# sreeramkannan/Shannon

Hardware: AMD Instinct MI355X
Metric: reads/sec k-mer->graph->path-decompose, 2x100bp k=25 (higher is better)
Workload: dtype u64

## Files before the change

### include/shannon_hip.h

```cpp
#ifndef SHANNON_HIP_H
#define SHANNON_HIP_H
#include <stdint.h>
#ifdef __cplusplus
extern "C" {
#endif

typedef struct shn_ctx shn_ctx;
typedef struct shn_reads shn_reads;
typedef struct shn_table shn_table;

#define SHN_OK 0
#define SHN_ERR_ARG -1
#define SHN_ERR_HIP -2
#define SHN_ERR_NOMEM -3
#define SHN_ERR_OVERFLOW -4
#define SHN_ERR_INTERNAL -5

#define SHN_ENC_ASCII 0
#define SHN_ENC_CODES 1

const char* shn_last_error(void);
const char* shn_version(void);

int shn_ctx_create(int device, void* stream, shn_ctx** out);
// ... 5 lines not shown
int shn_timer_reset(shn_ctx* ctx);
int shn_timer_ms(shn_ctx* ctx, int slot, double* ms, uint64_t* n_regions);
int shn_timer_bytes(shn_ctx* ctx, int slot, uint64_t* bytes);
const char* shn_timer_name(int slot);

int shn_reads_create(shn_ctx* ctx, const uint8_t* bytes, const uint64_t* offsets, uint64_t n_reads,
                     uint32_t fixed_len, int enc, shn_reads** out);
void shn_reads_destroy(shn_reads* r);
uint64_t shn_reads_count(const shn_reads* r);
uint64_t shn_reads_total_bases(const shn_reads* r);
uint32_t shn_reads_max_len(const shn_reads* r);
uint64_t shn_reads_n_invalid(const shn_reads* r);

int shn_string_windows(const uint8_t* text, const uint64_t* off, uint64_t n_strings, int k, uint64_t* keys_out, uint8_t* rows_out);

int shn_gather_rows(const uint8_t* src, uint64_t n_src_rows, uint64_t row_bytes, const int64_t* idx, uint64_t n, uint8_t* dst, int threads);
int shn_gather_segments(const uint8_t* src, const uint64_t* src_off, uint64_t n_src, const int64_t* order, uint64_t n, uint8_t* dst,
                        const uint64_t* dst_off, int threads);
int shn_fasta_records(const uint8_t* src, const uint64_t* src_off, uint64_t n_src, const int64_t* order, uint64_t n, const char* prefix,
                      uint8_t* dst, uint64_t dst_cap, uint64_t* dst_len);

int shn_count_k1mers(shn_ctx* ctx, shn_reads* const* sets, int n_sets, int k1, int both_strands,
                     shn_table** out);
void shn_table_destroy(shn_table* t);
uint64_t shn_table_size(const shn_table* t);
uint64_t shn_table_total(const shn_table* t);
int shn_table_k(const shn_table* t);
int shn_table_canonical(const shn_table* t);
int shn_table_download(shn_ctx* ctx, const shn_table* t, uint64_t* keys, uint32_t* counts);
int shn_table_dump(shn_ctx* ctx, const shn_table* t, uint32_t lower, uint64_t* keys, uint32_t* counts,
                   uint64_t* n);
int shn_table_filter_lower(shn_ctx* ctx, const shn_table* t, uint32_t lower, shn_table** out);
int shn_table_device_ptrs(const shn_table* t, void** keys, void** counts);
int shn_table_lookup(shn_ctx* ctx, const shn_table* t, const uint64_t* keys, uint64_t n, uint32_t* counts);

int shn_table_from_pairs(shn_ctx* ctx, const void* dev_keys, const void* dev_counts, uint64_t n, int k1,
                         int canonical, shn_table** out);
int shn_table_merge_rc(shn_ctx* ctx, const shn_table* fwd, const shn_table* other, shn_table** out);
int shn_table_shard(shn_ctx* ctx, const shn_table* t, int n_ranks, uint64_t* per_rank, void* dev_keys_out,
                    void* dev_counts_out);
int shn_table_shard_mode(shn_ctx* ctx, const shn_table* t, int n_ranks, int mode, uint64_t* per_rank, void* dev_keys_out,
                         void* dev_counts_out);

typedef struct shn_ext shn_ext;
int shn_extend(shn_ctx* ctx, const shn_table* t, uint32_t min_weight, int max_iterations, shn_ext** out);
void shn_ext_destroy(shn_ext* e);
uint64_t shn_ext_n_walks(const shn_ext* e);
int shn_ext_iterations(const shn_ext* e);
uint64_t shn_ext_total_steps(const shn_ext* e);
uint64_t shn_ext_wave_steps(const shn_ext* e);
uint64_t shn_ext_fresh_steps(const shn_ext* e);
int shn_ext_dense_rounds(const shn_ext* e);
uint64_t shn_ext_settled_walks(const shn_ext* e);
int shn_ext_digests(const shn_ext* e, uint64_t* out );
uint64_t shn_debug_counter(int which);
int shn_debug_alloc(shn_ctx* ctx, uint64_t bytes, void** out);
void shn_debug_free(shn_ctx* ctx, void* p);
int shn_debug_fill(shn_ctx* ctx, void* p, uint64_t n_words, uint32_t value, uint32_t spin);
int shn_debug_read(shn_ctx* ctx, const void* p, uint64_t n_words, uint32_t* host_out);
int shn_ext_stats(shn_ctx* ctx, const shn_ext* e, uint32_t* n_right, uint32_t* n_left, uint64_t* tot_weight);
int shn_ext_stats_range(shn_ctx* ctx, const shn_ext* e, uint64_t lo, uint64_t n, uint32_t* n_right, uint32_t* n_left, uint64_t* tot_weight);
typedef void (*shn_block_cb)(void* user, shn_ext* ext, uint64_t lo, uint64_t hi, int status);
void shn_ext_set_block_callback(shn_block_cb cb, void* user);
int shn_ext_emit(shn_ctx* ctx, const shn_ext* e, const uint32_t* ranks, uint64_t n_sel, const uint64_t* offsets,
                 uint8_t* bases_out);
int shn_ext_weights(shn_ctx* ctx, const shn_ext* e, const uint64_t* keys, uint64_t n, uint32_t* weights);
// ... 165 lines not shown
```

### shannon_amd/_lib.py

```python
import ctypes as C
import os

_PKG = os.path.dirname(os.path.abspath(__file__))
LIB_PATH = os.environ.get("SHN_HIP_LIB") or os.path.join(_PKG, "libshannon_hip.so")
_lib = None

u8p, u32p, u64p, dblp = C.POINTER(C.c_uint8), C.POINTER(C.c_uint32), C.POINTER(C.c_uint64), C.POINTER(C.c_double)
vp, vpp = C.c_void_p, C.POINTER(C.c_void_p)

SIGNATURES = {
    "shn_last_error": (C.c_char_p, []),
    "shn_version": (C.c_char_p, []),
    "shn_ctx_create": (C.c_int, [C.c_int, vp, vpp]),
    "shn_ctx_destroy": (None, [vp]),
    "shn_ctx_sync": (C.c_int, [vp]),
    "shn_ctx_fork": (C.c_int, [vp, vpp]),
    "shn_ctx_own_workspaces": (C.c_int, [vp]),
    "shn_timer_reset": (C.c_int, [vp]),
    "shn_timer_ms": (C.c_int, [vp, C.c_int, dblp, u64p]),
    "shn_timer_bytes": (C.c_int, [vp, C.c_int, u64p]),
    "shn_timer_name": (C.c_char_p, [C.c_int]),
    "shn_reads_create": (C.c_int, [vp, vp, vp, C.c_uint64, C.c_uint32, C.c_int, vpp]),
    "shn_reads_destroy": (None, [vp]),
    "shn_reads_count": (C.c_uint64, [vp]),
    "shn_reads_total_bases": (C.c_uint64, [vp]),
    "shn_reads_max_len": (C.c_uint32, [vp]),
    "shn_reads_n_invalid": (C.c_uint64, [vp]),
    "shn_string_windows": (C.c_int, [vp, vp, C.c_uint64, C.c_int, vp, vp]),
    "shn_gather_rows": (C.c_int, [vp, C.c_uint64, C.c_uint64, vp, C.c_uint64, vp, C.c_int]),
    "shn_gather_segments": (C.c_int, [vp, vp, C.c_uint64, vp, C.c_uint64, vp, vp, C.c_int]),
    "shn_fasta_records": (C.c_int, [vp, vp, C.c_uint64, vp, C.c_uint64, C.c_char_p, vp, C.c_uint64, u64p]),
    "shn_count_k1mers": (C.c_int, [vp, vpp, C.c_int, C.c_int, C.c_int, vpp]),
    "shn_table_destroy": (None, [vp]),
    "shn_table_size": (C.c_uint64, [vp]),
    "shn_table_total": (C.c_uint64, [vp]),
    "shn_table_k": (C.c_int, [vp]),
    "shn_table_canonical": (C.c_int, [vp]),
    "shn_table_download": (C.c_int, [vp, vp, vp, vp]),
    "shn_table_dump": (C.c_int, [vp, vp, C.c_uint32, vp, vp, u64p]),
    "shn_table_filter_lower": (C.c_int, [vp, vp, C.c_uint32, vpp]),
    "shn_table_device_ptrs": (C.c_int, [vp, vpp, vpp]),
    "shn_table_lookup": (C.c_int, [vp, vp, vp, C.c_uint64, vp]),
    "shn_table_from_pairs": (C.c_int, [vp, vp, vp, C.c_uint64, C.c_int, C.c_int, vpp]),
    "shn_table_merge_rc": (C.c_int, [vp, vp, vp, vpp]),
    "shn_table_shard": (C.c_int, [vp, vp, C.c_int, u64p, vp, vp]),
    "shn_table_shard_mode": (C.c_int, [vp, vp, C.c_int, C.c_int, u64p, vp, vp]),
    "shn_debug_cc_counters": (C.c_int, [u64p, C.c_int]),
    "shn_cc_create": (C.c_int, [vp, vp, C.c_int, C.c_int, vpp]),
    "shn_cc_destroy": (None, [vp]),
    "shn_cc_query_counts": (C.c_int, [vp, u64p]),
    "shn_cc_queries": (C.c_int, [vp, vp, vp]),
    "shn_cc_answer": (C.c_int, [vp, vp, vp, u64p, u64p, vp, u64p]),
    "shn_cc_solve": (C.c_int, [vp, vp, C.c_uint64, C.c_uint64, vp, vp, u64p]),
    "shn_cc_labels": (C.c_int, [vp, C.c_uint64, vp, vp, C.c_uint64, vp]),
    "shn_cc_owners": (C.c_int, [vp, vp, vp, vp, C.c_uint64, vp]),
    "shn_cc_shard": (C.c_int, [vp, vp, u64p, vp, vp]),
    "shn_table_create": (C.c_int, [vp, vp, vp, C.c_uint64, C.c_int, C.c_int, vpp]),
    "shn_probe_build": (C.c_int, [vp, vp, vp, C.c_uint64, vp, C.c_uint32, C.c_int, vpp]),
    "shn_probe_destroy": (None, [vp]),
    "shn_probe_table": (vp, [vp]),
    "shn_probe_n_sets": (C.c_uint32, [vp]),
    "shn_probe_n_members": (C.c_uint64, [vp]),
    "shn_probe_sets": (C.c_int, [vp, vp, vp]),
    "shn_route_reads": (C.c_int, [vp, vp, vp, C.c_int, vp, vp, vp, C.c_uint32, vpp]),
    "shn_route_reads_mode": (C.c_int, [vp, vp, vp, C.c_int, vp, vp, vp, C.c_uint32, C.c_int, vpp]),
    "shn_routes_destroy": (None, [vp]),
    "shn_routes_size": (C.c_uint64, [vp]),
    "shn_routes_download": (C.c_int, [vp, vp, vp, vp]),
    "shn_routes_bounds": (C.c_int, [vp, vp, C.c_uint32, C.c_uint32, vp, vp]),
    "shn_routes_download_range": (C.c_int, [vp, vp, C.c_uint64, C.c_uint64, vp]),
    "shn_lp_solve_batch": (C.c_int, [vp, C.c_uint32, vp, vp, vp, vp, vp, vp, C.c_uint64, vp]),
    "shn_lp_set_rule": (C.c_int, [vp, C.c_int]),
    "shn_lp_stats": (C.c_int, [vp, vp, C.c_int]),
    "shn_contig_graph": (C.c_int, [vp, vp, C.c_uint64, C.c_int, C.c_int, C.c_double, vp, u64p, vp, vp, vp, u64p]),
# ... 170 lines not shown
```

### shannon_amd/csrc/count.hip

```cpp
#include "common.h"
#include <mutex>
#include <atomic>
#include <thread>
#include <functional>
#include <cmath>
#include <algorithm>
#include <cstring>

#define BLK 256
#define CAP 1024
#define CAP_LIMIT 950
#define TARGET_BUCKET 640
#define TILE_IDS 65536
#define TILE_KEYS 32768
#define EMPTY_KEY 0xFFFFFFFFFFFFFFFFULL

#include "count_views.h"

#define bucket_of shn_bucket_of

template <bool CANON>
__device__ __forceinline__ bool gen_key(const ReadsView& v, uint64_t r, uint32_t pos, int k, uint64_t& key) {
  uint32_t len = v.len ? v.len[r] : v.fixed_len;
  if (pos + k > len) return false;
// ... 907 lines not shown
  ShnDevBufs bufs(s);
  uint32_t* d_flag = nullptr; uint64_t* d_pos = nullptr;
  HIP_TRY(bufs.get(&d_flag, (n + 1) * 4)); HIP_TRY(bufs.get(&d_pos, (n + 2) * 8));
  const dim3 grid((uint32_t)std::max<uint64_t>(1, std::min<uint64_t>(cdiv(n, 256), 1u << 20))), blk(256);
  if (n) hipLaunchKernelGGL(table_keep_kernel, grid, blk, 0, s, (const uint64_t*)t->d_keys, (const uint32_t*)t->d_counts, n, t->k, t->canonical, lower, d_flag);
  uint64_t kept = 0;
  if (n) { int rc = shn_device_scan_u32(ctx, d_flag, n, d_pos, &kept); if (rc) return rc; }
  else HIP_TRY(hipMemsetAsync(d_pos, 0, 16, s));
  shn_table* o = new shn_table();
  *o = *t;
  o->ctx = ctx; o->n = kept; o->d_keys = nullptr; o->d_counts = nullptr; o->d_bucket_off = nullptr;
#define TRYT(x) do { hipError_t _e = (x); if (_e != hipSuccess) { shn_table_destroy(o); return shn_fail(SHN_ERR_HIP, std::string(#x) + ": " + hipGetErrorString(_e)); } } while (0)
  TRYT(shn_dev_malloc(&o->d_keys, (kept + 1) * 8));
  TRYT(shn_dev_malloc(&o->d_counts, (kept + 1) * 4));
  TRYT(shn_dev_malloc(&o->d_bucket_off, nb1 * 8));
  if (n) hipLaunchKernelGGL(table_keep_scatter_kernel, grid, blk, 0, s, (const uint64_t*)t->d_keys, (const uint32_t*)t->d_counts, (const uint32_t*)d_flag,
                            (const uint64_t*)d_pos, n, o->d_keys, o->d_counts);
  hipLaunchKernelGGL(table_keep_boff_kernel, dim3((uint32_t)std::min<uint64_t>(cdiv(nb1, 256), 1u << 20)), blk, 0, s, (const uint64_t*)t->d_bucket_off, nb1,
                     (const uint64_t*)d_pos, o->d_bucket_off);
  TRYT(hipGetLastError());
  TRYT(hipStreamSynchronize(s));
#undef TRYT
  *out = o;
  return SHN_OK;
}

extern "C" int shn_table_device_ptrs(const shn_table* t, void** keys, void** counts) {
  if (!t) return shn_fail(SHN_ERR_ARG, "shn_table_device_ptrs: NULL table");
  if (keys) *keys = t->d_keys;
  if (counts) *counts = t->d_counts;
  return SHN_OK;
}

extern "C" int shn_table_lookup(shn_ctx* ctx, const shn_table* t, const uint64_t* keys, uint64_t n, uint32_t* counts) {
  if (!ctx || !t || (!keys && n) || (!counts && n)) return shn_fail(SHN_ERR_ARG, "shn_table_lookup: NULL argument");
  if (!n) return SHN_OK;
  SHN_ENTER(ctx);
  hipStream_t s = ctx->stream; shn_use_stream(s);
  uint64_t* dq; uint32_t* dc;
  HIP_TRY(shn_hip_malloc(&dq, n * 8));
  HIP_TRY(shn_hip_malloc(&dc, n * 4));
  HIP_TRY(hipMemcpyAsync(dq, keys, n * 8, hipMemcpyHostToDevice, s));
  {
    TimerRegion tr(ctx, T_LOOKUP);
    hipLaunchKernelGGL(lookup_kernel, dim3((uint32_t)cdiv(n, 256)), dim3(256), 0, s, shn_tab_idx(t), t->d_counts, dq, n, dc);
  }
  HIP_TRY(hipMemcpyAsync(counts, dc, n * 4, hipMemcpyDeviceToHost, s));
  HIP_TRY(hipStreamSynchronize(s));
  hipFree(dq); hipFree(dc);
  return SHN_OK;
}

__global__ void sum_counts_kernel(const uint32_t* __restrict__ c, uint64_t n, unsigned long long* __restrict__ out) {
  unsigned long long a = 0;
  for (uint64_t i = (uint64_t)blockIdx.x * blockDim.x + threadIdx.x; i < n; i += (uint64_t)gridDim.x * blockDim.x) a += c[i];
  for (int o = 32; o > 0; o >>= 1) a += __shfl_down(a, o, 64);
  if ((threadIdx.x & 63) == 0 && a) atomicAdd(out, a);
}

__global__ void table_rc_concat_kernel(const uint64_t* __restrict__ ka, const uint32_t* __restrict__ ca, uint64_t na, const uint64_t* __restrict__ kb,
                                       const uint32_t* __restrict__ cb, uint64_t nb, int k, uint64_t* __restrict__ keys, uint32_t* __restrict__ cnts) {
  for (uint64_t i = (uint64_t)blockIdx.x * blockDim.x + threadIdx.x; i < na + nb; i += (uint64_t)gridDim.x * blockDim.x) {
    if (i < na) { keys[i] = ka[i]; cnts[i] = ca[i]; }
    else { keys[i] = shn_revcomp(kb[i - na], k); cnts[i] = cb[i - na]; }
  }
}
// ... 156 lines not shown
```

### shannon_amd/csrc/extend.hip

```cpp
#include "common.h"
#include <cstring>
#include <vector>
#include <time.h>
#include <cstdio>
#include <cstdlib>
#include <algorithm>

#define EBLK 256
#define WBLK 64
#define UNCLAIMED 0xFFFFFFFFu
#define NONE32 0xFFFFFFFFu
#define UNCLAIMED64 0xFFFFFFFFFFFFFFFFULL
#define NOHINT_WORD 0xFFFFFFFFu
#define LONG_WALK 8
#define MEMO_MIN 1
#define PROMOTE_STEPS 16
typedef unsigned long long u64;
#define CLAIM(rank, pos) (((u64)(rank) << 32) | (u64)(uint32_t)(pos))
#define RANK(c) ((uint32_t)((c) >> 32))
#define POS(c) ((uint32_t)(c))

struct Adj4 { int32_t v[4]; };
struct __attribute__((aligned(64))) Rec {
  Adj4 R;
// ... 81 lines not shown
#define FD_SLOTS 10
#define FD_PER_LINE 4
#define FD_HOPS 4
#define FD_PAL 0x80000000u
__device__ __forceinline__ uint64_t fd_bucket(const TabIdx& T, uint64_t key, uint64_t n_lines) {
  const uint64_t h = shn_mix64(key);
  if (!T.layout) return __umul64hi(h, n_lines);
  const uint32_t b = shn_tab_bucket(T, key);
  const uint64_t lo = T.boff[b], hi = T.boff[b + 1];
  return lo / FD_PER_LINE + b + __umul64hi(h, (hi - lo) / FD_PER_LINE + 1);
}
__device__ __forceinline__ uint64_t fd_line_in_bucket(const TabIdx& T, uint32_t b, uint64_t key) {
  const uint64_t lo = T.boff[b], hi = T.boff[b + 1];
  return lo / FD_PER_LINE + b + __umul64hi(shn_mix64(key), (hi - lo) / FD_PER_LINE + 1);
}
__device__ __forceinline__ uint64_t xcd_block(int on) {
  const uint32_t g8 = gridDim.x & ~7u;
  if (!on || blockIdx.x >= g8) return blockIdx.x;
  return (uint64_t)(blockIdx.x & 7u) * (g8 >> 3) + (blockIdx.x >> 3);
}
__global__ void fd_build_kernel(const TabIdx T, const uint8_t* __restrict__ flags, uint64_t n,
                                unsigned long long* __restrict__ lines, uint64_t n_lines, int xcd) {
  const uint64_t* __restrict__ tkeys = T.keys;
  const uint64_t i = xcd_block(xcd) * blockDim.x + threadIdx.x;
  if (i >= n) return;
  const uint8_t f = flags[i];
  if (f & 2) return;
  const uint64_t key = tkeys[i];
  unsigned long long* line = lines + fd_bucket(T, key, n_lines) * 16;
  for (int hop = 0; hop < FD_HOPS; hop++, line += 16) {
    const uint32_t slot = atomicAdd((uint32_t*)line + 30, 1u);
    if (slot < FD_SLOTS) { line[slot] = key; ((uint32_t*)line)[20 + slot] = (uint32_t)i | ((f & 1) ? FD_PAL : 0u); break; }
  }
}
__device__ __forceinline__ uint64_t shfl_u64(uint64_t x, int src) {
  return ((uint64_t)(uint32_t)__shfl((int)(uint32_t)(x >> 32), src, 64) << 32) | (uint64_t)(uint32_t)__shfl((int)(uint32_t)x, src, 64);
}
__device__ __forceinline__ uint32_t fd_match(ulonglong2 v, const unsigned long long* __restrict__ lines, uint64_t line, uint64_t key, int p, int g0,
                                             const TabIdx& T, const uint8_t* __restrict__ flags) {
  for (int hop = 0;; hop++) {
    const bool ok = p < 5 && key != 0;
    const unsigned long long m0 = (__ballot(ok && v.x == key) >> g0) & 0xFFULL, m1 = (__ballot(ok && v.y == key) >> g0) & 0xFFULL;
    if (m0 | m1) {
      const int slot = m0 ? 2 * (__ffsll((long long)m0) - 1) : 2 * (__ffsll((long long)m1) - 1) + 1;
      const uint32_t w = (slot & 2) ? ((slot & 1) ? (uint32_t)(v.y >> 32) : (uint32_t)v.y) : ((slot & 1) ? (uint32_t)(v.x >> 32) : (uint32_t)v.x);
      return (uint32_t)__shfl((int)w, g0 + 5 + (slot >> 2), 64);
    }
    const uint32_t cnt = (uint32_t)__shfl((int)(uint32_t)(v.y >> 0), g0 + 7, 64) ;
    if (cnt <= FD_SLOTS || key == 0) return 0xFFFFFFFFu;
    if (hop == FD_HOPS - 1) break;
    line++;
    v = ((const ulonglong2*)(lines + line * 16))[p];
  }
  const int64_t j = shn_tab_find(T, key);
  if (j < 0) return 0xFFFFFFFFu;
  const uint8_t fj = flags[j];
  return (fj & 2) ? 0xFFFFFFFFu : ((uint32_t)j | ((fj & 1) ? FD_PAL : 0u));
}

struct __attribute__((aligned(16))) Quad { uint32_t a, b, c, d; };
#ifndef SHN_REC_PIPE
#define SHN_REC_PIPE 0
#endif

#if SHN_REC_PIPE
#define REC_KERNEL_ATTR __attribute__((amdgpu_waves_per_eu(5, 5)))
// ... 1236 lines not shown
    uint8_t* dst = out_bases + out_off[t];
    const uint64_t str = oriented_string(tkeys, (uint32_t)y, k);
    if (pos == 0) for (int j = 0; j < k; j++) dst[nl + j] = "ACGT"[(str >> (2 * (k - 1 - j))) & 3];
    else if (pos <= nr) dst[nl + k + (pos - 1)] = "ACGT"[str & 3];
    else dst[nl - 1 - (pos - nr - 1)] = "ACGT"[(str >> (2 * (k - 1))) & 3];
    n_wrote++;
  }
  __shared__ unsigned long long blk[2];
  if (threadIdx.x < 2) blk[threadIdx.x] = 0;
  __syncthreads();
  if (n_wrote) atomicAdd(&blk[0], (unsigned long long)n_wrote);
  if (n_stray) atomicAdd(&blk[1], (unsigned long long)n_stray);
  __syncthreads();
  if (threadIdx.x < 2 && blk[threadIdx.x]) atomicAdd(&counters[threadIdx.x], blk[threadIdx.x]);
}

__global__ void shard_select_kernel(const uint32_t* __restrict__ lab, const uint8_t* __restrict__ owner_root, uint64_t n, uint32_t my_rank,
                                    uint32_t* __restrict__ sel) {
  uint64_t i = (uint64_t)blockIdx.x * blockDim.x + threadIdx.x;
  if (i < n) sel[i] = owner_root[lab[i]] == my_rank ? 1u : 0u;
}
__global__ void shard_compact_kernel(const uint64_t* __restrict__ keys, const uint32_t* __restrict__ counts, const uint32_t* __restrict__ sel,
                                     const uint64_t* __restrict__ pos, uint64_t n, uint64_t* __restrict__ okeys, uint32_t* __restrict__ ocounts) {
  uint64_t i = (uint64_t)blockIdx.x * blockDim.x + threadIdx.x;
  if (i < n && sel[i]) { okeys[pos[i]] = keys[i]; ocounts[pos[i]] = counts[i]; }
}
__global__ void shard_offsets_kernel(const uint64_t* __restrict__ boff, uint64_t n_buckets, const uint64_t* __restrict__ pos,
                                     uint64_t* __restrict__ oboff) {
  uint64_t b = (uint64_t)blockIdx.x * blockDim.x + threadIdx.x;
  if (b <= n_buckets) oboff[b] = pos[boff[b]];
}

static int build_fine_dict(shn_ctx* ctx, const shn_table* t, const uint8_t* d_flags, unsigned long long** lines_out, uint64_t* n_lines_out,
                           void* room = nullptr);
static inline uint64_t fine_dict_lines(const shn_table* t) { return t->n / FD_PER_LINE + 1 + (t->layout ? t->n_buckets + 1 : 0) + FD_HOPS; }
static int component_shard(shn_ctx* ctx, const shn_table* t, int world, int rank, shn_table** out) {
  hipStream_t s = ctx->stream; shn_use_stream(s);
  const uint64_t n = t->n;
  uint32_t* d_weight = nullptr; uint8_t* d_flags = nullptr;
  unsigned long long* lines = nullptr;
  uint64_t n_lines = 0;
  shn_table* sub = nullptr;
  auto cleanup = [&]() { if (d_weight) shn_dev_free(d_weight); if (d_flags) shn_dev_free(d_flags); if (lines) shn_dev_free(lines); };
#define TRYS(x) do { hipError_t _e = (x); if (_e != hipSuccess) { cleanup(); if (sub) shn_table_destroy(sub); \
      return shn_fail(SHN_ERR_HIP, std::string(#x) + ": " + hipGetErrorString(_e)); } } while (0)
  TRYS(shn_dev_malloc(&d_weight, (n + 1) * 4));
  TRYS(shn_dev_malloc(&d_flags, n + 1));
  hipLaunchKernelGGL(ext_prepare_kernel, dim3((uint32_t)cdiv(n, 256)), dim3(256), 0, s, t->d_keys, t->d_counts, n, t->k, t->canonical, d_weight, d_flags);
  { int rca = build_fine_dict(ctx, t, d_flags, &lines, &n_lines); if (rca) { cleanup(); return rca; } }
  void *pl, *po, *pz, *pb, *pc, *pp;
  const uint32_t big_cap = 1u << 16;
  int rc;
  if ((rc = shn_ws(ctx)[14].get((n + 1) * 4, &pl)) || (rc = shn_ws(ctx)[15].get(n + 1, &po)) || (rc = shn_ws(ctx)[16].get((n + 1) * 4, &pz)) ||
      (rc = shn_ws(ctx)[17].get((size_t)big_cap * 9 + 64, &pb)) || (rc = shn_ws(ctx)[13].get(2048, &pc)) || (rc = shn_ws(ctx)[9].get((2 * n + 2) * 8, &pp))) { cleanup(); return rc; }
  uint32_t* d_lab = (uint32_t*)pl; uint8_t* d_owner_root = (uint8_t*)po;
  uint32_t* d_size = (uint32_t*)pz;
  uint32_t* d_big_root = (uint32_t*)pb; uint32_t* d_big_size = d_big_root + big_cap; uint8_t* d_big_owner = (uint8_t*)(d_big_size + big_cap);
  unsigned long long* d_cnt = (unsigned long long*)pc;
  uint64_t* d_pos = (uint64_t*)pp;
  TRYS(hipMemsetAsync(d_cnt, 0, 2048, s));
  hipLaunchKernelGGL(cc_init_kernel, dim3((uint32_t)cdiv(n, 256)), dim3(256), 0, s, d_lab, n);
  { TimerRegion t1(ctx, T_EXT_PREP);
    hipLaunchKernelGGL(cc_edges_kernel, dim3((uint32_t)std::min<uint64_t>(cdiv(n * 8, 256), 1u << 22)), dim3(256), 0, s, shn_tab_idx(t),
                       d_flags, n, t->k, t->canonical, d_lab, (const unsigned long long*)lines, n_lines, cc_half_mode()); }
  hipLaunchKernelGGL(cc_flatten_kernel, dim3((uint32_t)cdiv(n, 256)), dim3(256), 0, s, d_lab, n);
  TRYS(hipMemsetAsync(d_size, 0, (n + 1) * 4, s));
  hipLaunchKernelGGL(cc_sample_kernel, dim3((uint32_t)cdiv(cdiv(n, 64), 256)), dim3(256), 0, s, d_lab, n, d_size);
  hipLaunchKernelGGL(cc_owner_kernel, dim3((uint32_t)cdiv(n, 256)), dim3(256), 0, s, d_lab, d_size, n, (uint32_t)world, d_owner_root,
// ... 13 lines not shown
    std::vector<uint64_t> load(world, 0);
    std::vector<uint8_t> bo(nb);
    for (uint32_t j : ord) {
      int best = 0;
      for (int w = 1; w < world; w++) if (load[w] < load[best]) best = w;
      bo[j] = (uint8_t)best;
      load[best] += bs[j];
    }
    TRYS(hipMemcpyAsync(d_big_owner, bo.data(), nb, hipMemcpyHostToDevice, s));
    hipLaunchKernelGGL(cc_assign_kernel, dim3((uint32_t)cdiv(nb, 256)), dim3(256), 0, s, d_big_root, d_big_owner, (uint32_t)nb, d_owner_root);
  }
  uint32_t* d_sel = d_size;
  hipLaunchKernelGGL(shard_select_kernel, dim3((uint32_t)cdiv(n, 256)), dim3(256), 0, s, d_lab, d_owner_root, n, (uint32_t)rank, d_sel);
  uint64_t n_sub = 0;
  if ((rc = shn_device_scan_u32(ctx, d_sel, n, d_pos, &n_sub))) { cleanup(); return rc; }
  sub = new shn_table();
  memset(sub, 0, sizeof(*sub));
  sub->ctx = t->ctx; sub->device = t->device; sub->k = t->k; sub->canonical = t->canonical; sub->n = n_sub; sub->total = 0;
  sub->bits = t->bits; sub->n_buckets = t->n_buckets; sub->layout = t->layout; sub->sk_m = t->sk_m;
  TRYS(shn_dev_malloc(&sub->d_keys, (n_sub + 1) * 8));
  TRYS(shn_dev_malloc(&sub->d_counts, (n_sub + 1) * 4));
  TRYS(shn_dev_malloc(&sub->d_bucket_off, (t->n_buckets + 1) * 8));
  hipLaunchKernelGGL(shard_compact_kernel, dim3((uint32_t)cdiv(n, 256)), dim3(256), 0, s, t->d_keys, t->d_counts, d_sel, d_pos, n, sub->d_keys, sub->d_counts);
  hipLaunchKernelGGL(shard_offsets_kernel, dim3((uint32_t)cdiv(t->n_buckets + 1, 256)), dim3(256), 0, s, t->d_bucket_off, t->n_buckets, d_pos, sub->d_bucket_off);
  TRYS(hipStreamSynchronize(s));
  TRYS(hipGetLastError());
#undef TRYS
  cleanup();
  *out = sub;
  return SHN_OK;
}

static int build_fine_dict(shn_ctx* ctx, const shn_table* t, const uint8_t* d_flags, unsigned long long** lines_out, uint64_t* n_lines_out,
                           void* room) {
  hipStream_t s = ctx->stream; shn_use_stream(s);
  const uint64_t n = t->n;
  const uint64_t n_lines = fine_dict_lines(t);
  unsigned long long* lines = (unsigned long long*)room;
  hipError_t e = lines ? hipSuccess : shn_dev_malloc(&lines, n_lines * 128);
  if (e == hipSuccess) e = hipMemsetAsync(lines, 0, n_lines * 128, s);
  if (e != hipSuccess) { if (lines && !room) shn_dev_free(lines); return shn_fail(SHN_ERR_HIP, std::string("build_fine_dict: ") + hipGetErrorString(e)); }
  static const int xcd_map = getenv("SHN_XCD_MAP") && getenv("SHN_XCD_MAP")[0] == '1';
  if (n) hipLaunchKernelGGL(fd_build_kernel, dim3((uint32_t)cdiv(n, 256)), dim3(256), 0, s, shn_tab_idx(t), d_flags, n, lines, n_lines - FD_HOPS, xcd_map);
  *lines_out = lines; *n_lines_out = n_lines - FD_HOPS;
  return SHN_OK;
}

struct shn_cc {
  shn_ctx* ctx; const shn_table* t; int world, rank, device;
  uint8_t* d_flags; uint32_t* d_lab;
  unsigned long long* d_cnt;
  uint32_t* d_bc; uint64_t* d_pos;
  uint32_t q_grid;
  uint64_t per_rank[64];
};
#define CC_GRID 2048

__device__ __forceinline__ uint64_t cc_which_key(uint64_t str, int p, int half, int k, uint64_t mask, int canonical, bool* skip) {
  const uint64_t b = (uint64_t)(p & 3);
  uint64_t key;
  *skip = false;
  if (half == 0) key = (p & 4) ? ((str >> 2) | (b << (2 * (k - 1)))) : (((str << 2) | b) & mask);
  else if (p & 4) { *skip = (str & 3) == b; key = (str & ~3ULL) | b; }
  else { const int sh = 2 * (k - 1); *skip = ((str >> sh) & 3) == b; key = (str & ~(3ULL << sh)) | (b << sh); }
  if (canonical) { const uint64_t rc = shn_revcomp(key, k); if (rc < key) key = rc; }
  return key;
}

template <bool WRITE>
__global__ void cc_query_kernel(const uint64_t* __restrict__ tkeys, const uint8_t* __restrict__ flags, uint64_t n, int k, int canonical,
                                int world, int rank, const uint32_t* __restrict__ lab, unsigned long long* __restrict__ total,
                                uint32_t* __restrict__ block_count, const uint64_t* __restrict__ pos,
                                uint64_t* __restrict__ qk, uint32_t* __restrict__ ql) {
  __shared__ uint32_t lh[64];
  __shared__ uint64_t lbase[64];
  if (threadIdx.x < 64) {
// ... 392 lines not shown

extern "C" int shn_extend(shn_ctx* ctx, const shn_table* t, uint32_t min_weight, int max_iterations, shn_ext** out) {
  return shn_extend_sharded(ctx, t, min_weight, max_iterations, 1, 0, out);
}

extern "C" int shn_extend_sharded(shn_ctx* ctx, const shn_table* t, uint32_t min_weight, int max_iterations, int world, int rank,
                                  shn_ext** out) {
  if (!ctx || !t || !out) return shn_fail(SHN_ERR_ARG, "shn_extend: NULL argument");
  if (world < 1 || world > 255 || rank < 0 || rank >= world) return shn_fail(SHN_ERR_ARG, "shn_extend_sharded: bad world/rank");
  if (2 * t->n >= 0x7FFFFFFFULL) return shn_fail(SHN_ERR_ARG, "shn_extend: table too large for 31-bit oriented ids");
  SHN_ENTER(ctx);
  shn_stage_begin(ctx);
  hipStream_t s = ctx->stream; shn_use_stream(s);
  if (world > 1 && t->n) {
    shn_table* sub = nullptr;
    int rcs;
    { TimerRegion treg(ctx, T_EXTEND); rcs = component_shard(ctx, t, world, rank, &sub); }
    if (rcs) return rcs;
    rcs = shn_extend_sharded(ctx, sub, min_weight, max_iterations, 1, 0, out);
    if (rcs) { shn_table_destroy(sub); return rcs; }
    (*out)->owned_table = sub;
    return SHN_OK;
  }
  TimerRegion treg(ctx, T_EXTEND);
  shn_ext* e = new shn_ext();
  memset(e, 0, sizeof(*e));
  e->ctx = ctx; e->device = ctx->device; e->k = t->k; e->n = t->n; e->min_weight = min_weight; e->table = t;
  uint64_t n = t->n;
  if (max_iterations <= 0) max_iterations = 100000;
#define TRYE(x) do { hipError_t _e = (x); if (_e != hipSuccess) { shn_ext_destroy(e); \
      return shn_fail(SHN_ERR_HIP, std::string(#x) + ": " + hipGetErrorString(_e)); } } while (0)
  TRYE(shn_dev_malloc(&e->d_weight, (n + 1) * 4));
  TRYE(shn_dev_malloc(&e->d_flags, n + 1));
  TRYE(shn_dev_malloc(&e->d_rec, (2 * n + 1) * sizeof(Rec)));
  const uint64_t claim_words = (2 * n + 4 + 31) & ~31ULL;
  { u64* both = nullptr;
    TRYE(shn_dev_malloc(&both, std::max<uint64_t>(2 * claim_words * 8, fine_dict_lines(t) * 128)));
    e->d_claim = both; e->d_claim2 = both + claim_words; }
  if (n) {
    TimerRegion t1(ctx, T_EXT_PREP);
    hipLaunchKernelGGL(ext_prepare_kernel, dim3((uint32_t)cdiv(n, 256)), dim3(256), 0, s, t->d_keys, t->d_counts, n, t->k,
                       t->canonical, e->d_weight, e->d_flags);
    {
      unsigned long long* lines = nullptr;
      uint64_t n_lines = 0;
      { int rca = build_fine_dict(ctx, t, e->d_flags, &lines, &n_lines, e->d_claim); if (rca) { shn_ext_destroy(e); return rca; } }
      static const bool rec_lds = getenv("SHN_REC_LDS") && getenv("SHN_REC_LDS")[0] == '1';
      if (t->layout == 1 && rec_lds && t->n_buckets / REC_G + 1 < 0x7FFFFFFFULL) {
        TimerRegion ta(ctx, T_EXT_ADJ);
        hipLaunchKernelGGL(ext_records_lds_kernel, dim3((uint32_t)cdiv(t->n_buckets, REC_G)), dim3(256), 0, s, shn_tab_idx(t), e->d_flags, e->d_weight,
                           (uint64_t)t->n_buckets, t->k, t->canonical, e->d_rec, (const unsigned long long*)lines,
                           getenv("SHN_REC_ABLATE") ? atoi(getenv("SHN_REC_ABLATE")) : 0);
      } else
      { TimerRegion ta(ctx, T_EXT_ADJ);
        hipLaunchKernelGGL(ext_records_kernel, dim3((uint32_t)std::min<uint64_t>(cdiv(n * 8, 256), 1u << 22)), dim3(256), 0, s, shn_tab_idx(t),
                           e->d_flags, e->d_weight, n, t->k, t->canonical, e->d_rec, (const unsigned long long*)lines, n_lines,
                           (getenv("SHN_XCD_MAP") && getenv("SHN_XCD_MAP")[0] == '1') ? 1 : 0); }
      (void)lines;
    }
    TRYE(hipGetLastError());
  }
  void *pk, *pv, *pk2, *pv2, *pc;
  int rc;
  if ((rc = shn_ws(ctx)[13].get(2048, &pc))) { shn_ext_destroy(e); return rc; }
  unsigned long long* d_cnt = (unsigned long long*)pc;
  TRYE(hipMemsetAsync(d_cnt, 0, 2048, s));
  const uint64_t n_sblk = cdiv(n, 1024);
  uint32_t* d_bcnt = nullptr; uint64_t* d_bbase = nullptr;
  struct SeedScratch { uint32_t** a; uint64_t** b; ~SeedScratch() { if (*a) shn_dev_free(*a); if (*b) shn_dev_free(*b); } } seed_scratch{&d_bcnt, &d_bbase};
  TRYE(shn_dev_malloc(&d_bcnt, (n_sblk + 1) * 4));
  TRYE(shn_dev_malloc(&d_bbase, (n_sblk + 2) * 8));
  if (n) hipLaunchKernelGGL(ext_seed_kernel, dim3((uint32_t)n_sblk), dim3(1024), 0, s, t->d_keys, e->d_weight, e->d_flags, n,
                            t->k, t->canonical, min_weight, d_bcnt, (const uint64_t*)nullptr, (uint64_t*)nullptr, (uint32_t*)nullptr);
  uint64_t ns = 0;
  if (n && (rc = shn_device_scan_u32(ctx, d_bcnt, n_sblk, d_bbase, &ns))) { shn_ext_destroy(e); return rc; }
  if ((rc = shn_ws(ctx)[9].get((ns + 2) * 8, &pk)) || (rc = shn_ws(ctx)[10].get((ns + 2) * 4, &pv)) ||
      (rc = shn_ws(ctx)[11].get((ns + 2) * 8, &pk2)) || (rc = shn_ws(ctx)[12].get((ns + 2) * 4, &pv2))) { shn_ext_destroy(e); return rc; }
  uint64_t* skeys = (uint64_t*)pk; uint32_t* svals = (uint32_t*)pv;
  if (n) hipLaunchKernelGGL(ext_seed_kernel, dim3((uint32_t)n_sblk), dim3(1024), 0, s, t->d_keys, e->d_weight, e->d_flags, n,
// ... 630 lines not shown
```

### shannon_amd/device.py

```python
import ctypes as C
import numpy as np
from . import _lib

ENC_ASCII, ENC_CODES = 0, 1
ALPHA = "ACGT"
ALPHA_BYTES = np.frombuffer(b"ACGTN", dtype=np.uint8)


class Context(object):
    def __init__(self, device=0, stream=None, own_workspaces=False):
        self.h = C.c_void_p()
        _lib.check(_lib.lib().shn_ctx_create(int(device), C.c_void_p(stream or 0), C.byref(self.h)))
        self.device = device
        if own_workspaces:
            _lib.check(_lib.lib().shn_ctx_own_workspaces(self.h))

    def sync(self):
        _lib.check(_lib.lib().shn_ctx_sync(self.h))

    def timer_reset(self):
        _lib.check(_lib.lib().shn_timer_reset(self.h))

    def timers(self):
        out = {}
# ... 179 lines not shown
        return bool(_lib.lib().shn_table_canonical(self.h))

    def download(self):
        n = len(self)
        keys = np.empty(n, dtype=np.uint64)
        cnts = np.empty(n, dtype=np.uint32)
        _lib.check(_lib.lib().shn_table_download(self.ctx.h, self.h, keys.ctypes.data, cnts.ctypes.data))
        return keys, cnts

    def dump(self, lower=1):
        n = C.c_uint64(0)
        _lib.check(_lib.lib().shn_table_dump(self.ctx.h, self.h, lower, None, None, C.byref(n)))
        keys = np.empty(n.value, dtype=np.uint64)
        cnts = np.empty(n.value, dtype=np.uint32)
        _lib.check(_lib.lib().shn_table_dump(self.ctx.h, self.h, lower, keys.ctypes.data, cnts.ctypes.data, C.byref(n)))
        return keys[:n.value], cnts[:n.value]

    def filter_lower(self, lower):
        h = C.c_void_p()
        _lib.check(_lib.lib().shn_table_filter_lower(self.ctx.h, self.h, int(lower), C.byref(h)))
        return Table(self.ctx, h)

    def lookup(self, keys):
        keys = np.ascontiguousarray(keys, dtype=np.uint64)
        out = np.zeros(len(keys), dtype=np.uint32)
        _lib.check(_lib.lib().shn_table_lookup(self.ctx.h, self.h, keys.ctypes.data, len(keys), out.ctypes.data))
        return out

    def device_ptrs(self):
        k, c = C.c_void_p(), C.c_void_p()
        _lib.check(_lib.lib().shn_table_device_ptrs(self.h, C.byref(k), C.byref(c)))
        return k.value, c.value

    def shard(self, n_ranks, dev_keys_ptr, dev_counts_ptr):
        per = np.zeros(n_ranks, dtype=np.uint64)
        _lib.check(_lib.lib().shn_table_shard(self.ctx.h, self.h, n_ranks, per.ctypes.data_as(_lib.u64p),
                                              C.c_void_p(dev_keys_ptr), C.c_void_p(dev_counts_ptr)))
        return per

    def shard_by_minimizer(self, n_ranks, dev_keys_ptr, dev_counts_ptr):
        per = np.zeros(n_ranks, dtype=np.uint64)
        _lib.check(_lib.lib().shn_table_shard_mode(self.ctx.h, self.h, n_ranks, 1, per.ctypes.data_as(_lib.u64p),
                                                   C.c_void_p(dev_keys_ptr), C.c_void_p(dev_counts_ptr)))
        return per

    @classmethod
    def from_pairs(cls, ctx, dev_keys_ptr, dev_counts_ptr, n, k1, canonical):
        h = C.c_void_p()
        _lib.check(_lib.lib().shn_table_from_pairs(ctx.h, C.c_void_p(dev_keys_ptr), C.c_void_p(dev_counts_ptr), n, k1,
                                                   1 if canonical else 0, C.byref(h)))
        return cls(ctx, h)

    def close(self):
        if self.h:
            _lib.lib().shn_table_destroy(self.h)
            self.h = C.c_void_p()

    def __del__(self):
        try:
            self.close()
        except Exception:
            pass


class ComponentShards(object):

# ... 100 lines not shown
```

Baseline: 68.99 million.

## Build fine dictionary in LDS windows per bucket group instead of global atomics

Replaces the global-atomic fine-dictionary build, and its full memset, with a kernel that fills 128-line windows in shared memory for each group of buckets and then streams them out. This also zeroes the lines as they are written. Oversized groups and per-line slot overflow are sent to chunk lists, which a zero kernel and a global-atomic insert kernel then handle. The goal is to cut global atomic traffic and the separate memset, at the cost of repeated key scans per window, extra launches and scratch space reused from the rec buffer. It also adds a bucket-offsets query API for inspection.

```diff
diff --git a/include/shannon_hip.h b/include/shannon_hip.h
--- a/include/shannon_hip.h
+++ b/include/shannon_hip.h
@@ -61,6 +61,7 @@
                    uint64_t* n);
 int shn_table_filter_lower(shn_ctx* ctx, const shn_table* t, uint32_t lower, shn_table** out);
 int shn_table_device_ptrs(const shn_table* t, void** keys, void** counts);
+int shn_table_bucket_offsets(shn_ctx* ctx, const shn_table* t, uint64_t* n_buckets, int* layout, uint64_t* offsets);
 int shn_table_lookup(shn_ctx* ctx, const shn_table* t, const uint64_t* keys, uint64_t n, uint32_t* counts);
 
 int shn_table_from_pairs(shn_ctx* ctx, const void* dev_keys, const void* dev_counts, uint64_t n, int k1,
diff --git a/shannon_amd/_lib.py b/shannon_amd/_lib.py
--- a/shannon_amd/_lib.py
+++ b/shannon_amd/_lib.py
@@ -40,6 +40,7 @@
     "shn_table_dump": (C.c_int, [vp, vp, C.c_uint32, vp, vp, u64p]),
     "shn_table_filter_lower": (C.c_int, [vp, vp, C.c_uint32, vpp]),
     "shn_table_device_ptrs": (C.c_int, [vp, vpp, vpp]),
+    "shn_table_bucket_offsets": (C.c_int, [vp, vp, vp, vp, vp]),
     "shn_table_lookup": (C.c_int, [vp, vp, vp, C.c_uint64, vp]),
     "shn_table_from_pairs": (C.c_int, [vp, vp, vp, C.c_uint64, C.c_int, C.c_int, vpp]),
     "shn_table_merge_rc": (C.c_int, [vp, vp, vp, vpp]),
diff --git a/shannon_amd/csrc/count.hip b/shannon_amd/csrc/count.hip
--- a/shannon_amd/csrc/count.hip
+++ b/shannon_amd/csrc/count.hip
@@ -963,6 +963,19 @@
   return SHN_OK;
 }
 
+extern "C" int shn_table_bucket_offsets(shn_ctx* ctx, const shn_table* t, uint64_t* n_buckets, int* layout, uint64_t* offsets) {
+  if (!ctx || !t) return shn_fail(SHN_ERR_ARG, "shn_table_bucket_offsets: NULL argument");
+  SHN_ENTER(ctx);
+  if (n_buckets) *n_buckets = t->n_buckets;
+  if (layout) *layout = t->layout;
+  if (offsets) {
+    hipStream_t s = ctx->stream;
+    HIP_TRY(hipMemcpyAsync(offsets, t->d_bucket_off, (t->n_buckets + 1) * 8, hipMemcpyDeviceToHost, s));
+    HIP_TRY(hipStreamSynchronize(s));
+  }
+  return SHN_OK;
+}
+
 extern "C" int shn_table_lookup(shn_ctx* ctx, const shn_table* t, const uint64_t* keys, uint64_t n, uint32_t* counts) {
   if (!ctx || !t || (!keys && n) || (!counts && n)) return shn_fail(SHN_ERR_ARG, "shn_table_lookup: NULL argument");
   if (!n) return SHN_OK;
diff --git a/shannon_amd/csrc/extend.hip b/shannon_amd/csrc/extend.hip
--- a/shannon_amd/csrc/extend.hip
+++ b/shannon_amd/csrc/extend.hip
@@ -137,6 +137,88 @@
     const uint32_t slot = atomicAdd((uint32_t*)line + 30, 1u);
     if (slot < FD_SLOTS) { line[slot] = key; ((uint32_t*)line)[20 + slot] = (uint32_t)i | ((f & 1) ? FD_PAL : 0u); break; }
   }
+}
+#define FDL_W 128
+#define FDL_MAXW 8
+#define FDL_GMAX 8
+#define FDL_CHUNK 4096
+#define FDL_GRID 1024
+struct FdChunk { uint64_t start; uint32_t len, pad; };
+struct FdScratch { uint32_t* cnt; FdChunk* zlist; FdChunk* klist; uint32_t* over; };
+__global__ __launch_bounds__(256) void fd_build_lds_kernel(const TabIdx T, const uint8_t* __restrict__ flags, uint64_t n_buckets, uint32_t G,
+                                                           uint4* __restrict__ lines, uint64_t n_lines_total, const FdScratch S) {
+  __shared__ uint4 win[FDL_W * 8];
+  __shared__ uint64_t sboff[FDL_GMAX + 1];
+  __shared__ uint32_t sbase[2];
+  const uint64_t B0 = (uint64_t)blockIdx.x * G;
+  const uint32_t g = (uint32_t)(n_buckets - B0 < G ? n_buckets - B0 : G);
+  if (threadIdx.x <= g) sboff[threadIdx.x] = T.boff[B0 + threadIdx.x];
+  for (uint32_t idx = threadIdx.x; idx < FDL_W * 8; idx += blockDim.x) win[idx] = uint4{0u, 0u, 0u, 0u};
+  __syncthreads();
+  const uint64_t klo = sboff[0], khi = sboff[g];
+  const uint64_t A = klo / FD_PER_LINE + B0;
+  const uint64_t E = B0 + g == n_buckets ? n_lines_total : khi / FD_PER_LINE + B0 + g;
+  const uint64_t nl = E - A;
+  if (nl > (uint64_t)FDL_MAXW * FDL_W) {
+    const uint64_t nz = (nl + FDL_CHUNK - 1) / FDL_CHUNK, nk = (khi - klo + FDL_CHUNK - 1) / FDL_CHUNK;
+    if (threadIdx.x == 0) { sbase[0] = atomicAdd(&S.cnt[0], (uint32_t)nz); sbase[1] = atomicAdd(&S.cnt[1], (uint32_t)nk); }
+    __syncthreads();
+    for (uint64_t c = threadIdx.x; c < nz; c += blockDim.x) {
+      const uint64_t left = nl - c * FDL_CHUNK;
+      S.zlist[sbase[0] + c] = FdChunk{A + c * FDL_CHUNK, (uint32_t)(left < FDL_CHUNK ? left : FDL_CHUNK), 0u};
+    }
+    for (uint64_t c = threadIdx.x; c < nk; c += blockDim.x) {
+      const uint64_t left = khi - klo - c * FDL_CHUNK;
+      S.klist[sbase[1] + c] = FdChunk{klo + c * FDL_CHUNK, (uint32_t)(left < FDL_CHUNK ? left : FDL_CHUNK), 0u};
+    }
+    return;
+  }
+  for (uint64_t wlo = A; wlo < E; wlo += FDL_W) {
+    const uint32_t nlw = (uint32_t)(E - wlo < FDL_W ? E - wlo : FDL_W);
+    for (uint64_t t = klo + threadIdx.x; t < khi; t += blockDim.x) {
+      const uint8_t f = flags[t];
+      if (f & 2) continue;
+      const uint64_t key = T.keys[t];
+      uint32_t j = 0;
+      for (uint32_t q = 1; q < g; q++) j += sboff[q] <= t ? 1u : 0u;
+      const uint64_t lo = sboff[j], hi = sboff[j + 1];
+      const uint64_t line = lo / FD_PER_LINE + B0 + j + __umul64hi(shn_mix64(key), (hi - lo) / FD_PER_LINE + 1);
+      if (line < wlo || line - wlo >= nlw) continue;
+      uint32_t* L = (uint32_t*)&win[(line - wlo) * 8];
+      const uint32_t slot = atomicAdd(&L[30], 1u);
+      if (slot < FD_SLOTS) { ((unsigned long long*)L)[slot] = key; L[20 + slot] = (uint32_t)t | ((f & 1) ? FD_PAL : 0u); }
+      else S.over[atomicAdd(&S.cnt[2], 1u)] = (uint32_t)t;
+    }
+    __syncthreads();
+    for (uint32_t idx = threadIdx.x; idx < nlw * 8; idx += blockDim.x) { lines[wlo * 8 + idx] = win[idx]; win[idx] = uint4{0u, 0u, 0u, 0u}; }
+    __syncthreads();
+  }
+}
+__global__ void fd_zero_kernel(uint4* __restrict__ lines, const FdScratch S) {
+  const uint32_t nz = S.cnt[0];
+  for (uint32_t c = blockIdx.x; c < nz; c += gridDim.x) {
+    const FdChunk ch = S.zlist[c];
+    for (uint32_t idx = threadIdx.x; idx < ch.len * 8; idx += blockDim.x) lines[ch.start * 8 + idx] = uint4{0u, 0u, 0u, 0u};
+  }
+}
+__device__ __forceinline__ void fd_insert(const TabIdx& T, const uint8_t* __restrict__ flags, unsigned long long* __restrict__ lines, uint64_t n_lines,
+                                          uint64_t i, int hop) {
+  const uint8_t f = flags[i];
+  if (f & 2) return;
+  const uint64_t key = T.keys[i];
+  unsigned long long* line = lines + (fd_bucket(T, key, n_lines) + hop) * 16;
+  for (; hop < FD_HOPS; hop++, line += 16) {
+    const uint32_t slot = atomicAdd((uint32_t*)line + 30, 1u);
+    if (slot < FD_SLOTS) { line[slot] = key; ((uint32_t*)line)[20 + slot] = (uint32_t)i | ((f & 1) ? FD_PAL : 0u); break; }
+  }
+}
+__global__ void fd_insert_kernel(const TabIdx T, const uint8_t* __restrict__ flags, unsigned long long* __restrict__ lines, uint64_t n_lines, const FdScratch S) {
+  const uint32_t nk = S.cnt[1], no = S.cnt[2];
+  for (uint32_t c = blockIdx.x; c < nk; c += gridDim.x) {
+    const FdChunk ch = S.klist[c];
+    for (uint32_t t = threadIdx.x; t < ch.len; t += blockDim.x) fd_insert(T, flags, lines, n_lines, ch.start + t, 0);
+  }
+  for (uint32_t j = blockIdx.x * blockDim.x + threadIdx.x; j < no; j += gridDim.x * blockDim.x) fd_insert(T, flags, lines, n_lines, S.over[j], 1);
 }
 __device__ __forceinline__ uint64_t shfl_u64(uint64_t x, int src) {
   return ((uint64_t)(uint32_t)__shfl((int)(uint32_t)(x >> 32), src, 64) << 32) | (uint64_t)(uint32_t)__shfl((int)(uint32_t)x, src, 64);
@@ -1439,8 +1521,12 @@
 }
 
 static int build_fine_dict(shn_ctx* ctx, const shn_table* t, const uint8_t* d_flags, unsigned long long** lines_out, uint64_t* n_lines_out,
-                           void* room = nullptr);
+                           void* room = nullptr, void* scratch = nullptr);
 static inline uint64_t fine_dict_lines(const shn_table* t) { return t->n / FD_PER_LINE + 1 + (t->layout ? t->n_buckets + 1 : 0) + FD_HOPS; }
+static inline uint64_t fd_list_cap(uint64_t x) { return x / 512 + 16; }
+static inline uint64_t fine_dict_scratch(const shn_table* t) {
+  return 64 + (fd_list_cap(fine_dict_lines(t)) + fd_list_cap(t->n)) * sizeof(FdChunk) + (t->n + 16) * 4;
+}
 static int component_shard(shn_ctx* ctx, const shn_table* t, int world, int rank, shn_table** out) {
   hipStream_t s = ctx->stream; shn_use_stream(s);
   const uint64_t n = t->n;
@@ -1520,16 +1606,36 @@
 }
 
 static int build_fine_dict(shn_ctx* ctx, const shn_table* t, const uint8_t* d_flags, unsigned long long** lines_out, uint64_t* n_lines_out,
-                           void* room) {
+                           void* room, void* scratch) {
   hipStream_t s = ctx->stream; shn_use_stream(s);
   const uint64_t n = t->n;
   const uint64_t n_lines = fine_dict_lines(t);
+  const char* how = getenv("SHN_FD_BUILD");
+  const uint64_t per_bucket = t->n_buckets ? n / FD_PER_LINE / t->n_buckets + 1 : 1;
+  const uint32_t G = (uint32_t)std::max<uint64_t>(1, std::min<uint64_t>(std::min<uint64_t>(FDL_GMAX, t->n_buckets), (FDL_W / 2) / per_bucket));
+  const bool lds = t->layout == 1 && n && t->n_buckets && !(how && !strcmp(how, "atomic")) && cdiv(t->n_buckets, G) < 0x7FFFFFFFULL &&
+                   (!room || scratch);
   unsigned long long* lines = (unsigned long long*)room;
-  hipError_t e = lines ? hipSuccess : shn_dev_malloc(&lines, n_lines * 128);
-  if (e == hipSuccess) e = hipMemsetAsync(lines, 0, n_lines * 128, s);
+  hipError_t e = lines ? hipSuccess : shn_dev_malloc(&lines, n_lines * 128 + (lds ? fine_dict_scratch(t) : 0));
+  if (e == hipSuccess && !lds) e = hipMemsetAsync(lines, 0, n_lines * 128, s);
+  if (lds) {
+    char* sc = room ? (char*)scratch : (char*)lines + n_lines * 128;
+    FdScratch S;
+    S.cnt = (uint32_t*)sc;
+    S.zlist = (FdChunk*)(sc + 64);
+    S.klist = S.zlist + fd_list_cap(n_lines);
+    S.over = (uint32_t*)(S.klist + fd_list_cap(n));
+    if (e == hipSuccess) e = hipMemsetAsync(S.cnt, 0, 64, s);
+    if (e == hipSuccess) {
+      hipLaunchKernelGGL(fd_build_lds_kernel, dim3((uint32_t)cdiv(t->n_buckets, G)), dim3(256), 0, s, shn_tab_idx(t), d_flags, (uint64_t)t->n_buckets, G,
+                         (uint4*)lines, n_lines, S);
+      hipLaunchKernelGGL(fd_zero_kernel, dim3(FDL_GRID), dim3(256), 0, s, (uint4*)lines, S);
+      hipLaunchKernelGGL(fd_insert_kernel, dim3(FDL_GRID), dim3(256), 0, s, shn_tab_idx(t), d_flags, lines, n_lines - FD_HOPS, S);
+    }
+  }
   if (e != hipSuccess) { if (lines && !room) shn_dev_free(lines); return shn_fail(SHN_ERR_HIP, std::string("build_fine_dict: ") + hipGetErrorString(e)); }
   static const int xcd_map = getenv("SHN_XCD_MAP") && getenv("SHN_XCD_MAP")[0] == '1';
-  if (n) hipLaunchKernelGGL(fd_build_kernel, dim3((uint32_t)cdiv(n, 256)), dim3(256), 0, s, shn_tab_idx(t), d_flags, n, lines, n_lines - FD_HOPS, xcd_map);
+  if (n && !lds) hipLaunchKernelGGL(fd_build_kernel, dim3((uint32_t)cdiv(n, 256)), dim3(256), 0, s, shn_tab_idx(t), d_flags, n, lines, n_lines - FD_HOPS, xcd_map);
   *lines_out = lines; *n_lines_out = n_lines - FD_HOPS;
   return SHN_OK;
 }
@@ -1988,7 +2094,7 @@
       return shn_fail(SHN_ERR_HIP, std::string(#x) + ": " + hipGetErrorString(_e)); } } while (0)
   TRYE(shn_dev_malloc(&e->d_weight, (n + 1) * 4));
   TRYE(shn_dev_malloc(&e->d_flags, n + 1));
-  TRYE(shn_dev_malloc(&e->d_rec, (2 * n + 1) * sizeof(Rec)));
+  TRYE(shn_dev_malloc(&e->d_rec, std::max<uint64_t>((2 * n + 1) * sizeof(Rec), fine_dict_scratch(t))));
   const uint64_t claim_words = (2 * n + 4 + 31) & ~31ULL;
   { u64* both = nullptr;
     TRYE(shn_dev_malloc(&both, std::max<uint64_t>(2 * claim_words * 8, fine_dict_lines(t) * 128)));
@@ -2000,7 +2106,7 @@
     {
       unsigned long long* lines = nullptr;
       uint64_t n_lines = 0;
-      { int rca = build_fine_dict(ctx, t, e->d_flags, &lines, &n_lines, e->d_claim); if (rca) { shn_ext_destroy(e); return rca; } }
+      { int rca = build_fine_dict(ctx, t, e->d_flags, &lines, &n_lines, e->d_claim, e->d_rec); if (rca) { shn_ext_destroy(e); return rca; } }
       static const bool rec_lds = getenv("SHN_REC_LDS") && getenv("SHN_REC_LDS")[0] == '1';
       if (t->layout == 1 && rec_lds && t->n_buckets / REC_G + 1 < 0x7FFFFFFFULL) {
         TimerRegion ta(ctx, T_EXT_ADJ);
diff --git a/shannon_amd/device.py b/shannon_amd/device.py
--- a/shannon_amd/device.py
+++ b/shannon_amd/device.py
@@ -235,6 +235,13 @@
         _lib.check(_lib.lib().shn_table_device_ptrs(self.h, C.byref(k), C.byref(c)))
         return k.value, c.value
 
+    def bucket_offsets(self):
+        nb, lay = C.c_uint64(0), C.c_int(0)
+        _lib.check(_lib.lib().shn_table_bucket_offsets(self.ctx.h, self.h, C.byref(nb), C.byref(lay), None))
+        off = np.zeros(nb.value + 1, dtype=np.uint64)
+        _lib.check(_lib.lib().shn_table_bucket_offsets(self.ctx.h, self.h, None, None, off.ctypes.data))
+        return lay.value, off
+
     def shard(self, n_ranks, dev_keys_ptr, dev_counts_ptr):
         per = np.zeros(n_ranks, dtype=np.uint64)
         _lib.check(_lib.lib().shn_table_shard(self.ctx.h, self.h, n_ranks, per.ctypes.data_as(_lib.u64p),
```

New measurement: 67.70 million. -1.9%, worse.
